# SerezD/vqvae-vqgan-pytorch-lightning

Measured on AMD Instinct MI355X. Metric: images/sec/node (256x256 bs=32/GPU) VQ-VAE train step, higher is better.
Workload: dtype bf16; 1 GPU; standard_vqvae cb=1024, 256x256 bs=32/GPU (encoder+VQ+decoder fwd/bwd + AdamW); yaml=example_confs/standard_vqvae.yaml, global_batch=32, parallelism=dp1, launch=hipGraph replay (fwd+bwd) + eager all-reduce + AdamW, deterministic=False

## Files before the change

### vqvae-vqgan-pytorch-lightning_amd/csrc/api.cpp

```cpp
#include <stdint.h>
#include <new>
#include "common.h"

extern "C" {

const char* vqk_status_str(int status) {
    switch (status) {
        case VQK_OK: return "ok";
        case VQK_ERR_SHAPE: return "unsupported or inconsistent shape";
        case VQK_ERR_DTYPE: return "unsupported dtype";
        case VQK_ERR_ALIGN: return "pointer is not 16-byte aligned";
        case VQK_ERR_LAUNCH: return "kernel launch failed";
        case VQK_ERR_ARG: return "bad argument";
        case VQK_ERR_WORKSPACE: return "workspace too small";
        default: return "unknown status";
    }
}

int vqk_version(void) { return 1; }
const char* vqk_arch(void) { return "gfx950"; }

}

struct vqk_ctx {
// ... 80 lines not shown
    {"FPROP_SPLITK", 0, 0},
    {"SK_BLOCKS", 0, 0},
    {"SK_MINSTEPS", 0, 0},
    {"SK_MAXMB", 0, 0},
    {"UPS_PHASE", 0, 0},
    {"WGRAD_BLOCKS", 0, 0},
    {"WGMX", 0, 0},
    {"WGRAD_GEN_BLOCKS", 0, 0},
    {"WGRAD_NO_PW16", 0, 0},
    {"WGRAD_NO_P16K", 0, 0},
    {"MX_HALF", 0, 0},
    {"MX_HALF_HW", 0, 0},
    {"UPFIRDN_TILE", 0, 0},
    {"GN_BLOCKS_REDUCE", 0, 0},
    {"GN_BLOCKS_APPLY", 0, 0},
    {"GN_NT_MB", 0, 0},
    {"GN_NO_SMALL", 0, 0},
    {"WGMX_COEF_E4", 0, 0},
    {"GN_CLUSTER_MAX_HW", 0, 0},
    {"COMM_CUS", 0, 0},
    {"MX_QUARTER", 0, 0},
    {"MX_S2", 0, 0},
    {"MX_S2_DGRAD_MIN", 0, 0},
    {"VQ_LDS", 0, 0},
    {"UPS_MERGE", 0, 0},
    {"TILE_QUEUE", 0, 0},
    {"X3_WL", 0, 0},
    {"X3_WGRAD_COEF_E4", 0, 0},
    {"X3_WGRAD_FOLD", 0, 0},
    {"X3_WGRAD_PHASE", 0, 0},
    {"X3_WGRAD_PHASE_CAP_PCT", 0, 0},
    {"X3_WGRAD_PHASE_COEF_E4", 0, 0},
    {"WGRAD_GROUP_LOAD_PCT", 0, 0},
    {"WGRAD_GROUP_MIN_PPS", 0, 0}
};
static constexpr int kTune = (int)(sizeof(g_tune) / sizeof(g_tune[0]));
TuneSlot* tune_slot(const char* name) {
    for (int i = 0; i < kTune; ++i)
        if (strcmp(g_tune[i].name, name) == 0) return &g_tune[i];
    abort();
}
}

extern "C" int vqk_set_tuning(const char* name, int value) {
    if (!name) return VQK_ERR_ARG;
    for (int i = 0; i < vqkd::kTune; ++i)
        if (strcmp(vqkd::g_tune[i].name, name) == 0) {
            __atomic_store_n(&vqkd::g_tune[i].value, value, __ATOMIC_RELAXED);
            __atomic_store_n(&vqkd::g_tune[i].is_set, 1, __ATOMIC_RELEASE);
            return VQK_OK;
        }
    return VQK_ERR_ARG;
}

extern "C" int vqk_reset_tuning(void) {
    for (int i = 0; i < vqkd::kTune; ++i) __atomic_store_n(&vqkd::g_tune[i].is_set, 0, __ATOMIC_RELAXED);
    return VQK_OK;
}

extern "C" int vqk_tuning_count(void) { return vqkd::kTune; }

extern "C" const char* vqk_tuning_name(int i) { return (i >= 0 && i < vqkd::kTune) ? vqkd::g_tune[i].name : nullptr; }
```

### vqvae-vqgan-pytorch-lightning_amd/csrc/conv.hip

```cpp
#include "conv_geom.h"
#include <type_traits>
#include <stdlib.h>
#include <math.h>

namespace {

using vqkd::ConvGeom;
using vqkd::xcd_remap;
using vqkd::pack_bf16x2;

__device__ __forceinline__ float epi_act(float v, int act) {
    if (act == 1) return tanhf(v);
    if (act == 2) return fmaxf(v, 0.0f);
    if (act == 3) return v > 0.0f ? v : 0.2f * v;
    return v;
}
__device__ __forceinline__ float epi_act_sel(float v, int act) {
    const float lo = act == 2 ? 0.0f : act == 3 ? 0.2f * v : v;
    return fmaxf(v, lo);
}


template <typename T> struct Mma;
template <> struct Mma<bf16_raw> {
// ... 975 lines not shown
                }
            }
        }
#pragma unroll
        for (int s5 = 0; s5 < 5; ++s5) a[s5] = an[s5];
    }
    if constexpr (STATS) {
        asm volatile("s_nop 3" : "+v"(sga), "+v"(sqa), "+v"(sgb), "+v"(sqb));
        sga += __shfl_xor(sga, 16, 64); sga += __shfl_xor(sga, 32, 64);
        sqa += __shfl_xor(sqa, 16, 64); sqa += __shfl_xor(sqa, 32, 64);
        sgb += __shfl_xor(sgb, 16, 64); sgb += __shfl_xor(sgb, 32, 64);
        sqb += __shfl_xor(sqb, 16, 64); sqb += __shfl_xor(sqb, 32, 64);
        if (lane < 16) {
            const int groups = g.cout >> 2;
            double* dst = g.gn_ws + ((int64_t)img_s * groups + ((cout_base >> 2) + 2 * lane)) * 2;
            atomicAdd(dst, (double)sga); atomicAdd(dst + 1, (double)sqa);
            atomicAdd(dst + 2, (double)sgb); atomicAdd(dst + 3, (double)sqb);
        }
    }
}

static thread_local int g_force_variant = CONV_VARIANT_AUTO;
#define g_det (vqkd::det_state().on)
#define g_det_ws (vqkd::det_state().ws)
#define g_det_ws_bytes (vqkd::det_state().bytes)
static thread_local int g_stream_blocks = 0;
static thread_local int g_wgrad_blocks = 0;

inline bool mx_shape_ok(const ConvGeom& g, int variant) {
    return VQK_TUNE("MX", 1) && variant != CONV_VARIANT_NO_MX && (g.cout & 127) == 0 && (g.cpt >> 2) >= 2 &&
           (int64_t)g.n * g.h_in * g.w_in * g.cin * 2 < 0x7fffffffLL && (int64_t)g.m * g.cout * 2 < 0x7fffffffLL;
}

inline bool mx_serves_1x1(const ConvGeom& g, int variant) {
    return mx_shape_ok(g, variant) && VQK_TUNE("MX_1X1", 1) && !g.ups;
}

inline int halo_twlog(const ConvGeom& g, int variant) {
    if ((g.ks != 3 && g.ks != 1) || (g.cpt % 8) != 0 || variant == CONV_VARIANT_IM2COL) return 0;
    if (g.ks == 1 && !mx_serves_1x1(g, variant)) return 0;
    const int prefer16 = VQK_TUNE("TW16", 0);
    if (prefer16 && (g.w % 16) == 0 && (g.h % 16) == 0) return 4;
    if ((g.w % 32) == 0 && (g.h % 8) == 0) return 5;
    if ((g.w % 16) == 0 && (g.h % 16) == 0) return 4;
    return 0;
}

inline bool fused_epilogue_serves(const ConvGeom& g, int variant) {
    return halo_twlog(g, variant) && (g.cout % 128) == 0 && variant != CONV_VARIANT_BREG && variant != CONV_VARIANT_PLAIN_WEIGHTS;
}

inline bool thin_f32_plain(const ConvGeom& g, int variant) {
    return g.ks == 3 && !g.ups && !g.zs && !g.sub && g.stride == 1 && g.pad == 1 && g.vh == g.h && g.vw == g.w &&
           variant != CONV_VARIANT_IM2COL;
}
inline bool thin_out_f32_serves(const ConvGeom& g, int variant) {
    return thin_f32_plain(g, variant) && g.cout == 4 && (g.cin % 16) == 0 && (g.h % 8) == 0 && (g.w % 32) == 0;
}
inline bool thin_in_f32_serves(const ConvGeom& g, int variant, bool has_res, int act) {
    return thin_f32_plain(g, variant) && g.cin == 4 && (g.cout == 64 || g.cout == 128 || g.cout == 256) && !has_res && act == 0 &&
           g.acc_scale == 1.0f && g.out_gain == 1.0f && g.w >= 4 && (g.w % 4) == 0 && (int64_t)(10) * (g.w + 2) * 16 <= 64 * 1024;
}

enum ConvForm : int {
    FORM_THIN_OUT_F32 = 0,
    FORM_THIN_IN_F32,
// ... 159 lines not shown
        launch_im2col<T, TO>(p, st, x, w, bias, res, y, zeros, g, act, skws);
        hipLaunchKernelGGL(conv_splitk_epilogue_kernel<TO>, dim3((unsigned)(((int64_t)g.m * g.cout / 4 + 255) / 256)), dim3(256), 0, st,
                           skws, bias, (const TO*)res, (TO*)y, g, act, p.splits);
        break;
    }
    default: return VQK_ERR_ARG;
    }
    if (hipGetLastError() != hipSuccess) return VQK_ERR_LAUNCH;
    return VQK_OK;
}

int launch_fprop_any(int dtype, int out_dtype, const void* x, const void* w, const float* bias, const void* res, void* y,
                     const void* zeros, const ConvGeom& g, int act, int wlayout, int variant, hipStream_t st) {
    if (dtype == VQK_F32 && out_dtype == VQK_F32) return launch_fprop<float, float>(x, w, bias, res, y, zeros, g, act, wlayout, variant, st);
    if (dtype == VQK_BF16 && out_dtype == VQK_BF16) return launch_fprop<bf16_raw, bf16_raw>(x, w, bias, res, y, zeros, g, act, wlayout, variant, st);
    if (dtype == VQK_BF16 && out_dtype == VQK_F32) return launch_fprop<bf16_raw, float>(x, w, bias, res, y, zeros, g, act, wlayout, variant, st);
    return VQK_ERR_DTYPE;
}

int make_geom(ConvGeom& g, int dtype, int n, int h_in, int w_in, int cin, int cout, int ksize, int ups) {
    if (dtype != VQK_F32 && dtype != VQK_BF16) return VQK_ERR_DTYPE;
    const int epc = dtype == VQK_F32 ? 4 : 8;
    if (n <= 0 || h_in <= 0 || w_in <= 0 || cin <= 0 || cout <= 0) return VQK_ERR_SHAPE;
    if (ksize != 1 && ksize != 3) return VQK_ERR_SHAPE;
    if (ups != 0 && ups != 1) return VQK_ERR_ARG;
    if (cin % epc) return VQK_ERR_SHAPE;
    g.n = n; g.h_in = h_in; g.w_in = w_in; g.h = h_in << ups; g.w = w_in << ups;
    g.cin = cin; g.cout = cout; g.ks = ksize; g.ups = ups;
    g.stride = 1; g.pad = ksize >> 1; g.zs = 0; g.vh = g.h; g.vw = g.w;
    g.acc_scale = 1.0f; g.out_gain = 1.0f; g.pool = 0; g.pool_scale = 1.0f;
    g.gn_ws = nullptr; g.gn_cpg = 0; g.gn_part_nblk = 0; g.gn_part_base = 0;
    g.act = 0; g.dy_pool = 0; g.tq = nullptr; g.tq_mode = 0; g.phase_rev = 0;
    g.ntap = ksize == 1 ? 1 : 9; g.tap_oy = g.tap_ox = 0; g.src_s = 1; g.src_a = g.src_b = 0; g.dst_s = 1; g.dst_a = g.dst_b = 0;
    g.tapw = 0; g.dst_h = g.dst_w = 0; g.s2 = 0; g.phase_mode = 0;
    g.fold = 0;
    const int64_t m = (int64_t)n * g.h * g.w;
    if (m > 0x7fffffff - 256) return VQK_ERR_SHAPE;
    g.m = (int)m;
    g.cpt = cin / epc;
    g.kchunks = ksize * ksize * g.cpt;
    g.wrow_chunks = g.kchunks; g.sub = 0;
    g.tiles_m = (g.m + 127) / 128;
    g.tiles_n = (cout + 127) / 128;
    return VQK_OK;
}

}

namespace vqkd {
int conv_make_geom(ConvGeom& g, int dtype, int n, int h_in, int w_in, int cin, int cout, int ksize, int ups) {
    return make_geom(g, dtype, n, h_in, w_in, cin, cout, ksize, ups);
}
int& conv_force_variant() { return g_force_variant; }
int& conv_wgrad_blocks() { return g_wgrad_blocks; }
}

extern "C" {

int vqk_conv_set_variant(int v) { g_force_variant = v; return VQK_OK; }
int vqk_conv_set_block_caps(int stream_blocks, int wgrad_blocks) {
    g_stream_blocks = stream_blocks; g_wgrad_blocks = wgrad_blocks;
    return VQK_OK;
}

static int conv_general(int dtype, const void* x, const void* w, const float* bias, const void* residual, void* y,
                        int out_dtype, int n, int h_in, int w_in, int cin, int cout, int ksize, int stride, int pad,
                        int mode, int h_out, int w_out, int act, float acc_scale, float out_gain, int wlayout,
// ... 178 lines not shown
        gx.gn_ws = gn_ws; gx.gn_cpg = cpg;
        return vqkd::launch_conv3x3_x3(x, w4, backward ? nullptr : bias, res, y, zeros, gx, 0, 0, vqk_stream(stream));
    }
    VQK_REQUIRE(!gn_ws || ((!backward || phase_rev) && groups > 0 && cout % groups == 0 && (cout / groups) % 4 == 0), VQK_ERR_SHAPE);
    VQK_REQUIRE(!res || (backward && phase_rev && vqk_aligned16(res)), VQK_ERR_ARG);
    ConvGeom g;
    const int rc = make_geom(g, dtype, n, h, w, cin, cout, 3, 0);
    if (rc) return rc;
    const int tw = halo_twlog(g, g_force_variant);
    const int mx_on = VQK_TUNE("MX", 1);
    const int ph_on = VQK_TUNE("UPS_PHASE", 1);
    VQK_REQUIRE(tw && mx_on && ph_on && (cout % 128) == 0 && (g.cpt >> 2) >= 2 && g_force_variant != CONV_VARIANT_NO_MX, VQK_ERR_SHAPE);
    VQK_REQUIRE((int64_t)4 * g.m * (backward ? cin : cout) * 2 < 0x7fffffffLL && (int64_t)g.m * (backward ? cout : cin) * 2 < 0x7fffffffLL,
                VQK_ERR_SHAPE);
    g.ntap = 4;
    const int64_t phase_elems = (int64_t)((cout + 127) / 128) * 128 * cin * 4;
    hipStream_t st = vqk_stream(stream);
    if (VQK_TUNE("UPS_MERGE", 1)) {
        ConvGeom gp = g;
        if (!backward) {
            gp.phase_mode = 1;
            gp.dst_s = 2;
            gp.phase_rev = phase_rev; gp.acc_scale = acc_scale;
            gp.gn_ws = gn_ws; gp.gn_cpg = gn_ws ? cout / groups : 0;
            if (gn_ws && g_det) { gp.gn_part_nblk = 4 * ((g.h * g.w) / 256); gp.gn_part_base = 0; }
        } else {
            gp.phase_mode = 2;
            gp.src_s = 2;
            gp.h_in = 2 * h; gp.w_in = 2 * w;
            gp.phase_rev = phase_rev; gp.acc_scale = acc_scale;
            gp.gn_ws = gn_ws; gp.gn_cpg = gn_ws ? cout / groups : 0;
            if (gn_ws && g_det) { gp.gn_part_nblk = (g.h * g.w) / 256; gp.gn_part_base = 0; }
        }
        return vqkd::launch_conv3x3_mx(x, w4, backward ? nullptr : bias, res, y, zeros, gp, tw, st);
    }
    for (int ph = 0; ph < 4; ++ph) {
        const int a = ph >> 1, b = ph & 1;
        ConvGeom gp = g;
        const void* res = nullptr;
        if (!backward) {
            gp.tap_oy = a; gp.tap_ox = b;
            gp.dst_s = 2; gp.dst_a = a; gp.dst_b = b;
            gp.gn_ws = gn_ws; gp.gn_cpg = gn_ws ? cout / groups : 0;
            if (gn_ws && g_det) { gp.gn_part_nblk = 4 * ((g.h * g.w) / 256); gp.gn_part_base = ph * ((g.h * g.w) / 256); }
        } else {
            gp.tap_oy = 1 - a; gp.tap_ox = 1 - b;
            gp.src_s = 2; gp.src_a = a; gp.src_b = b;
            gp.h_in = 2 * h; gp.w_in = 2 * w;
            res = ph ? y : nullptr;
        }
        const int r = vqkd::launch_conv3x3_mx(x, (const bf16_raw*)w4 + ph * phase_elems, backward ? nullptr : bias, res, y, zeros, gp, tw, st);
        if (r != VQK_OK) return r;
    }
    return VQK_OK;
}

static int s2_twlog(int h_out, int w_out, int pix) {
    if ((w_out % 32) == 0 && (h_out % (pix / 32)) == 0) return 5;
    if ((w_out % 16) == 0 && (h_out % (pix / 16)) == 0) return 4;
    return 0;
}

int vqk_conv2d_s2_supported(int dtype, int n, int h_out, int w_out, int cin, int cout, int backward) {
    if (dtype != VQK_BF16 || n <= 0 || h_out <= 0 || w_out <= 0 || cin <= 0 || cout <= 0) return 0;
    if (!VQK_TUNE("MX", 1) || !VQK_TUNE("MX_S2", 1) || g_force_variant == CONV_VARIANT_IM2COL || g_force_variant == CONV_VARIANT_NO_MX) return 0;
    const int64_t big = (int64_t)n * (2 * h_out + 1) * (2 * w_out + 1) * cin * 2, small = (int64_t)n * h_out * w_out * cout * 2;
    if (big >= 0x7fffffffLL || small >= 0x7fffffffLL) return 0;
    if (!backward) return (cin % 64) == 0 && (cout % 128) == 0 && s2_twlog(h_out, w_out, 128) != 0;
    return (cout % 64) == 0 && (cin % 128) == 0 && s2_twlog(h_out, w_out, 256) != 0 && w_out >= VQK_TUNE("MX_S2_DGRAD_MIN", 32);
}

int vqk_conv2d_s2_fprop(int dtype, const void* x, const void* wq, const float* bias, void* y, int n, int h_out, int w_out,
                        int cin, int cout, int act, float acc_scale, float out_gain, const void* zeros, void* stream) {
    VQK_REQUIRE(x && wq && y && zeros, VQK_ERR_ARG);
    VQK_REQUIRE(vqk_aligned16(x) && vqk_aligned16(wq) && vqk_aligned16(y), VQK_ERR_ALIGN);
    VQK_REQUIRE(act == 0 || act == 2 || act == 3, VQK_ERR_ARG);
    VQK_REQUIRE(vqk_conv2d_s2_supported(dtype, n, h_out, w_out, cin, cout, 0), VQK_ERR_SHAPE);
    ConvGeom g;
    const int rc = make_geom(g, dtype, n, h_out, w_out, cin, cout, 3, 0);
    if (rc) return rc;
    g.h_in = 2 * h_out + 1; g.w_in = 2 * w_out + 1;
    g.src_s = 2; g.s2 = 1;
    g.act = act; g.acc_scale = acc_scale; g.out_gain = out_gain;
// ... 132 lines not shown
```

### vqvae-vqgan-pytorch-lightning_amd/csrc/conv_geom.h

```cpp
#pragma once
#include "common.h"

namespace vqkd {

struct ConvGeom {
    int n, h_in, w_in, h, w, cin, cout, ks, ups;
    int stride, pad, zs, vh, vw;
    float acc_scale, out_gain;
    int pool;
    float pool_scale;
    int m;
    int sub, sub_py, sub_px, sub_h, sub_w, nkh, nkw, khl[2], kwl[2];
    int wrow_chunks;
    int cpt;
    int kchunks;
    int tiles_m, tiles_n;
    double* gn_ws;
    int gn_cpg;
    int gn_part_nblk, gn_part_base;
    int ntap, tap_oy, tap_ox, src_s, src_a, src_b, dst_s, dst_a, dst_b;
    int tapw, dst_h, dst_w, s2;
    int phase_mode;
    int phase_rev;
    int dy_pool;
    int act;
    int* tq;
    int tq_mode;
    int fold;
};

__device__ __forceinline__ int xcd_remap(int bid, int total) {
    const int q = total >> 3, r = total & 7, xcd = bid & 7, k = bid >> 3;
    return (xcd < r ? xcd * (q + 1) : r * (q + 1) + (xcd - r) * q) + k;
}

__device__ __forceinline__ unsigned pack_bf16x2(float a, float b) {
    typedef __attribute__((ext_vector_type(2))) float f32x2;
    typedef __attribute__((ext_vector_type(2))) __bf16 bf16x2_t;
    const f32x2 v = {a, b};
    return __builtin_bit_cast(unsigned, __builtin_convertvector(v, bf16x2_t));
}

int launch_conv3x3_mx(const void* x, const void* w, const float* bias, const void* res, void* y, const void* zeros,
                      const ConvGeom& g, int twlog, hipStream_t st);

int conv_make_geom(ConvGeom& g, int dtype, int n, int h_in, int w_in, int cin, int cout, int ksize, int ups);
}
enum ConvVariant : int {
    CONV_VARIANT_AUTO = -1,
    CONV_VARIANT_IM2COL = 0,
    CONV_VARIANT_HALO = 1,
    CONV_VARIANT_PLAIN_WEIGHTS = 2,
    CONV_VARIANT_BREG = 3,
    CONV_VARIANT_NO_HALF = 4,
    CONV_VARIANT_NO_MX = 5,
    CONV_VARIANT_MX = 6,
};
namespace vqkd {
int& conv_force_variant();
int& conv_wgrad_blocks();

bool conv3x3_x3_serves(const ConvGeom& g);
int launch_conv3x3_x3(const void* x, const void* w, const float* bias, const void* res, void* y, const void* zeros,
                      const ConvGeom& g, int act, int blocks_cap, hipStream_t st);
int launch_conv3x3_wgrad_x3(const void* x, const void* dy, float* dw, const ConvGeom& g, int blocks_cap, hipStream_t st);

int launch_conv3x3_thin_out_f32(const float* x, const float* w, const float* bias, const float* res, float* y, int n, int h, int wd,
                                int cin, int act, float acc_scale, float out_gain, hipStream_t st);
int launch_conv3x3_thin_in_f32(const float* x, const float* w, const float* bias, float* y, int n, int h, int wd, int cout, hipStream_t st);
int thin_wgrad_rows(int h, int w);
int launch_conv3x3_wgrad_thin_f32(int mode, const float* wide, const float* thin, float* dw, int n, int h, int w, int cw, float scale,
                                  hipStream_t st);

// ... 19 lines not shown
```

### vqvae-vqgan-pytorch-lightning_amd/csrc/conv_mx.hip

```cpp
#include "conv_geom.h"
#include <stdlib.h>

namespace {
using vqkd::ConvGeom;
using vqkd::pack_bf16x2;
using vqkd::xcd_remap;

#ifndef VQK_MX_RD
#define VQK_MX_RD 6
#endif
#ifndef VQK_MX_NT
#define VQK_MX_NT 2
#endif
#ifndef VQK_MX_HALO_AUX
#define VQK_MX_HALO_AUX 0
#endif
#ifndef VQK_MX_PRIO
#define VQK_MX_PRIO 0
#endif
#ifndef VQK_MX_PACE
#define VQK_MX_PACE 0
#endif
#ifndef VQK_MX_WL
#define VQK_MX_WL 0
#endif
#ifndef VQK_MX_JOUTER
#define VQK_MX_JOUTER 0
#endif
#ifndef VQK_MX_PIN
#define VQK_MX_PIN 1
#endif

#define SGB(mask, n) __builtin_amdgcn_sched_group_barrier(mask, n, 0)

__host__ __device__ constexpr int mx_tap_pix(bool s2, int tap, int twd, int hw2, int shp) {
    return s2 ? (((tap / 3) & 1) * 2 + ((tap % 3) & 1)) * shp + ((tap / 3) >> 1) * hw2 + ((tap % 3) >> 1)
              : (tap / twd) * hw2 + (tap % twd);
}

template <int TWLOG, bool POOL, int NTAP, int PIXELS = 256, int TAPW = 0, bool S2 = false>
__global__ __launch_bounds__(512, 2) void conv3x3_mx_kernel(const bf16_raw* __restrict__ x, const bf16_raw* __restrict__ wp,
                                                            const float* __restrict__ bias,
                                                            const bf16_raw* __restrict__ res, bf16_raw* __restrict__ y,
                                                            ConvGeom g) {
    constexpr int HM = NTAP == 1 ? 0 : 1;
    constexpr int PIX = PIXELS, TW = 1 << TWLOG, TH = PIX / TW;
    constexpr int HW2 = S2 ? TW + 1 : TW + 2 * HM;
    constexpr int SHP = (TH + 1) * (TW + 1);
    constexpr int HROWS = S2 ? 4 * SHP : (TH + 2 * HM) * HW2;
    constexpr int RS = 80;
    constexpr int PIECES = (HROWS * 5 + 63) / 64;
    constexpr int NBUF = S2 ? 2 : 3;
    constexpr int BUF = PIECES * 1024, STG = NBUF * BUF, SPITCH = 272, SCR = STG + PIX * SPITCH;
    constexpr int TQR = SCR + 1024;
    constexpr int TWD = TAPW ? TAPW : NTAP == 9 ? 3 : NTAP == 4 ? 2 : 1;
    constexpr int NI = VQK_MX_WL ? PIX / 32 : PIX / 64, NJ = VQK_MX_WL ? 1 : 2;
    constexpr int NQ = PIX / 16;
    static_assert(PIX == 256 || ((PIX == 128 || PIX == 64) && !POOL && NTAP == 9), "256-pixel tiles, or plain 128- / 64-pixel part tiles");
    constexpr int NPH = NTAP * 2;
    static_assert(NTAP == 9 || ((NTAP == 4 || NTAP == 2 || NTAP == 1) && !POOL), "3x3 taps, the 2x2 / 1x2 / 2x1 taps of a phase, or a 1x1 conv");
    static_assert(!S2 || (NTAP == 9 && !POOL && PIX == 128), "stride 2: 3x3 taps, 128-pixel tiles");
    static_assert(TAPW == 0 || (NTAP == 2 && (TAPW == 1 || TAPW == 2)), "TAPW names the orientation of a 2-tap window");
    constexpr int XS = (PIECES + 3) / 4;
    constexpr int OOB = (int)0x80000000;
    typedef bf16x8_t frag_t;
    typedef __attribute__((ext_vector_type(4))) unsigned int u32x4;
    typedef __attribute__((ext_vector_type(2))) unsigned int u32x2;
    extern __shared__ __attribute__((aligned(16))) char smem[];

    const int tid = threadIdx.x, lane = tid & 63;
    const int wave = __builtin_amdgcn_readfirstlane(tid >> 6);
    const int tiles_x = g.w >> TWLOG, tiles_y = g.h / TH;
    const int pmode = NTAP == 4 ? g.phase_mode : 0;
    const int total_tiles = g.n * tiles_y * tiles_x * g.tiles_n * (pmode == 1 ? 4 : 1);
    const int nch = g.cpt >> 2;
    const int nun = pmode == 2 ? 4 * nch : nch;
    const int grid = (int)gridDim.x, q8 = grid >> 3, r8 = grid & 7, xcd = (int)blockIdx.x & 7;
    const int cnt = q8 + (xcd < r8 ? 1 : 0);
    const int c0 = xcd < r8 ? xcd * (q8 + 1) : r8 * (q8 + 1) + (xcd - r8) * q8;
    const int vbid = c0 + ((int)blockIdx.x >> 3);
    if (vbid >= total_tiles) return;
    auto tile_of = [&](int k) -> int { const int j = k / cnt; return c0 + (k - j * cnt) + j * grid; };
    const int tqm = g.tq ? g.tq_mode : 0;
    volatile VQK_LDS int* const ring = (volatile VQK_LDS int*)(smem + TQR);
    auto next_id = [&](int j) -> int { return tqm ? __builtin_amdgcn_readfirstlane(ring[j & 7]) : vbid + j * grid; };
    const bool pro_sync = tqm == 2 || (tqm && nun < 4);

    struct TilePos { int img, py0, px0, nt, ph; };
    auto tile_pos = [&](int t) -> TilePos {
        TilePos tp;
        tp.nt = t % g.tiles_n; t /= g.tiles_n;
        tp.ph = 0;
        if (pmode == 1) { tp.ph = t & 3; t >>= 2; }
        const int txi = t % tiles_x; t /= tiles_x;
        const int tyi = t % tiles_y;
        tp.img = t / tiles_y; tp.py0 = tyi * TH; tp.px0 = txi * TW;
        return tp;
    };
    auto unit_barrier = [&]() { asm volatile("s_waitcnt lgkmcnt(0)\n\ts_barrier" ::: "memory"); };
    double* const gnws = g.gn_ws;

    if (wave < 4) {
        if (VQK_MX_PRIO) __builtin_amdgcn_s_setprio(VQK_MX_PRIO);
        const int wm = VQK_MX_WL ? 0 : wave >> 1, wn = VQK_MX_WL ? wave : wave & 1;
        const int p = lane & 31, kg = lane >> 5;
        unsigned abase[NI], sbase[NI];
#pragma unroll
        for (int i = 0; i < NI; ++i) {
            int ty, tx;
            if (TWLOG == 5) { ty = wm * NI + i; tx = p; }
            else { ty = wm * 2 * NI + 2 * i + (p >> 4); tx = p & 15; }
            abase[i] = (unsigned)(((ty + (pmode ? 0 : g.tap_oy)) * HW2 + tx + (pmode ? 0 : g.tap_ox)) * RS + kg * 16);
            sbase[i] = (unsigned)(STG + (ty * TW + tx) * SPITCH + (wn * (32 * NJ) + 4 * kg) * 2);
        }
        const int lane16 = lane * 16;
        const int phase_bytes = (g.cout >> 5) * nch * (NPH * 1024);
        const __amdgpu_buffer_rsrc_t wsrd = __builtin_amdgcn_make_buffer_rsrc(
            const_cast<bf16_raw*>(wp), 0, phase_bytes * (pmode ? 4 : 1), 0x00020000);
        auto unit_ph = [&](int key, int c) -> int { return pmode == 2 ? c / nch : (key >> 16); };
        auto unit_w = [&](int key, int c, int j) -> int {
            const int ph = unit_ph(key, c), cc = pmode == 2 ? c - ph * nch : c;
            const int wph = (NTAP == 4 && g.phase_rev) ? 3 - ph : ph;
            return wph * phase_bytes + (((key & 0xffff) * 4 + wn * NJ + j) * nch + cc) * (NPH * 1024);
        };
        auto phase_off = [&](int ph) -> int {
            const int a = ph >> 1, b = ph & 1;
            return pmode == 1 ? (a * HW2 + b) * RS : pmode == 2 ? ((1 - a) * HW2 + (1 - b)) * RS : 0;
        };
        auto tile_nt = [&](int t) -> int {
            return (t % g.tiles_n) | (pmode == 1 ? ((t / g.tiles_n) & 3) << 16 : 0);
        };
        auto wload = [&](int soff) -> frag_t {
            return __builtin_bit_cast(frag_t, __builtin_amdgcn_raw_buffer_load_b128(wsrd, lane16, soff, 0));
        };

        constexpr int RD = NTAP == 9 ? VQK_MX_RD : NTAP == 4 ? 4 : 2;
        static_assert(NPH % RD == 0, "weight ring depth must divide the phases of a unit");
        f32x16 acc[NI][NJ];
        frag_t bw[RD][NJ];
        int wcur[NJ];
        if (pro_sync) unit_barrier();
        const int t_first = tqm == 2 ? __builtin_amdgcn_readfirstlane(ring[0]) : vbid;
        if (t_first >= total_tiles) return;
        int cur_nt = tile_nt(t_first);
#pragma unroll
        for (int j = 0; j < NJ; ++j) wcur[j] = unit_w(cur_nt, 0, j);
#pragma unroll
        for (int d = 0; d < RD; ++d)
#pragma unroll
            for (int j = 0; j < NJ; ++j) bw[d][j] = wload(wcur[j] + d * 1024);
        unit_barrier();

        int tj = 0, c = 0, bi = 0, t_next = 0;
        for (;;) {
            if (c == nun - 2) t_next = next_id(tj + 1);
            const bool last_c = c == nun - 1, more = last_c && t_next < total_tiles;
            int nc = c + 1, nxt_nt = cur_nt;
            if (last_c) {
                if (more) { nc = 0; nxt_nt = tile_nt(t_next); }
                else nc = c;
            }
            int wnxt[NJ];
#pragma unroll
            for (int j = 0; j < NJ; ++j) wnxt[j] = unit_w(nxt_nt, nc, j);
            const char* lbase[NI];
#pragma unroll
            for (int i = 0; i < NI; ++i) lbase[i] = smem + bi * BUF + abase[i] + (NTAP == 4 ? phase_off(unit_ph(cur_nt, c)) : 0);

            frag_t a[2][NI];
#pragma unroll
            for (int i = 0; i < NI; ++i) a[0][i] = *reinterpret_cast<const frag_t*>(lbase[i]);
            __builtin_amdgcn_sched_barrier(0);
#pragma unroll
            for (int tap = 0; tap < NTAP; ++tap) {
                const int toff = mx_tap_pix(S2, tap, TWD, HW2, SHP) * RS;
#pragma unroll
                for (int ks = 0; ks < 2; ++ks) {
                    const bool reads = ks == 0 || tap < NTAP - 1;
                    const int ph = tap * 2 + ks;
                    if (ks == 0) {
#pragma unroll
                        for (int i = 0; i < NI; ++i) a[1][i] = *reinterpret_cast<const frag_t*>(lbase[i] + toff + 32);
                    } else if (tap < NTAP - 1) {
                        const int toff1 = mx_tap_pix(S2, tap + 1, TWD, HW2, SHP) * RS;
#pragma unroll
                        for (int i = 0; i < NI; ++i) a[0][i] = *reinterpret_cast<const frag_t*>(lbase[i] + toff1);
                    }
                    if (tap == 0 && ks == 0 && c == 0) {
                        const f32x16 zero = {0.f, 0.f, 0.f, 0.f, 0.f, 0.f, 0.f, 0.f, 0.f, 0.f, 0.f, 0.f, 0.f, 0.f, 0.f, 0.f};
#pragma unroll
                        for (int i = 0; i < NI; ++i)
#pragma unroll
                            for (int j = 0; j < NJ; ++j)
                                acc[i][j] = __builtin_amdgcn_mfma_f32_32x32x16_bf16(bw[ph % RD][j], a[ks][i], zero, 0, 0, 0);
                    } else if (VQK_MX_JOUTER) {
#pragma unroll
                        for (int j = 0; j < NJ; ++j)
#pragma unroll
                            for (int i = 0; i < NI; ++i)
                                acc[i][j] = __builtin_amdgcn_mfma_f32_32x32x16_bf16(bw[ph % RD][j], a[ks][i], acc[i][j], 0, 0, 0);
                    } else {
#pragma unroll
                        for (int i = 0; i < NI; ++i)
#pragma unroll
                            for (int j = 0; j < NJ; ++j)
                                acc[i][j] = __builtin_amdgcn_mfma_f32_32x32x16_bf16(bw[ph % RD][j], a[ks][i], acc[i][j], 0, 0, 0);
                    }
#pragma unroll
                    for (int j = 0; j < NJ; ++j) {
                        const int soff = (ph + RD >= NPH) ? wnxt[j] + (ph + RD - NPH) * 1024 : wcur[j] + (ph + RD) * 1024;
                        bw[ph % RD][j] = wload(soff);
                    }
                    if (VQK_MX_PIN) {
                        if (reads) {
#pragma unroll
                            for (int i = 0; i < NI; ++i) { SGB(0x008, 1); SGB(0x100, 1); }
                            if constexpr (NI * NJ - NI > 0) SGB(0x008, NI * NJ - NI);
                        } else {
                            SGB(0x008, NI * NJ);
                        }
                        SGB(0x020, NJ);
// ... 4 lines not shown
            if (c == nun - 1) {
#pragma unroll
                for (int i = 0; i < NI; ++i)
#pragma unroll
                    for (int j = 0; j < NJ; ++j)
#pragma unroll
                        for (int rq = 0; rq < 4; ++rq) {
                            const u32x2 o = {pack_bf16x2(acc[i][j][4 * rq], acc[i][j][4 * rq + 1]),
                                             pack_bf16x2(acc[i][j][4 * rq + 2], acc[i][j][4 * rq + 3])};
                            *reinterpret_cast<u32x2*>(smem + sbase[i] + (j * 32 + 8 * rq) * 2) = o;
                        }
            }
            unit_barrier();
            if (last_c) { if (!more) break; ++tj; }
            cur_nt = nxt_nt; c = nc;
            bi = bi == NBUF - 1 ? 0 : bi + 1;
#pragma unroll
            for (int j = 0; j < NJ; ++j) wcur[j] = wnxt[j];
        }
        return;
    }

    const int xt = tid - 256, xw = wave - 4;
    const __amdgpu_buffer_rsrc_t xsrd = __builtin_amdgcn_make_buffer_rsrc(
        const_cast<bf16_raw*>(x), 0, (int)((int64_t)g.n * g.h_in * g.w_in * g.cin * 2), 0x00020000);
    const int out_bytes = (int)((int64_t)g.n * g.dst_h * g.dst_w * g.cout * 2);
    const __amdgpu_buffer_rsrc_t rsrd = __builtin_amdgcn_make_buffer_rsrc(const_cast<bf16_raw*>(res), 0, res ? out_bytes : 0, 0x00020000);
    const __amdgpu_buffer_rsrc_t ysrd = __builtin_amdgcn_make_buffer_rsrc(y, 0, out_bytes >> (POOL ? 2 : 0), 0x00020000);

    int rel[XS], flg[XS];
#pragma unroll
    for (int sl = 0; sl < XS; ++sl) {
        const int s = (xw + 4 * sl) * 64 + lane;
        const int hp = s / 5, cp = s - hp * 5;
        if constexpr (S2) {
            const int sh = hp / SHP, q = hp - sh * SHP;
            const int hy = q / HW2, hx = q - hy * HW2, pa = sh >> 1, pb = sh & 1;
            rel[sl] = (((2 * hy + pa) * g.w_in + 2 * hx + pb) * g.cin + cp * 8) * 2;
            flg[sl] = (cp == 4 || hp >= HROWS || (pa && hy == TH) || (pb && hx == TW)) ? 16 : 0;
        } else {
            const int hy = hp / HW2, hx = hp - hy * HW2;
            rel[sl] = (((((hy - HM) * g.src_s) >> g.ups) * g.w_in + (((hx - HM) * g.src_s) >> g.ups)) * g.cin + cp * 8) * 2;
            flg[sl] = (HM && hy == 0 ? 1 : 0) | (HM && hy == TH + 1 ? 2 : 0) | (HM && hx == 0 ? 4 : 0) | (HM && hx == TW + 1 ? 8 : 0) |
                      ((cp == 4 || hp >= HROWS) ? 16 : 0);
        }
    }
    auto issue_halo = [&](const TilePos& tp, int cu, int bufi) {
        const int uph = pmode == 2 ? cu / nch : 0, c = pmode == 2 ? cu - uph * nch : cu;
        const int sa = pmode == 2 ? (uph >> 1) : g.src_a, sb = pmode == 2 ? (uph & 1) : g.src_b;
        const int base = (((tp.img * g.h_in + ((tp.py0 * g.src_s + sa) >> g.ups)) * g.w_in + ((tp.px0 * g.src_s + sb) >> g.ups)) * g.cin + c * 32) * 2;
        const int tb = S2 ? 16 : ((tp.py0 == 0 ? 1 : 0) | (tp.py0 + TH == g.h ? 2 : 0) | (tp.px0 == 0 ? 4 : 0) | (tp.px0 + TW == g.w ? 8 : 0) | 16);
#pragma unroll
        for (int sl = 0; sl < XS; ++sl) {
            if (xw + 4 * sl < PIECES) {
                const int off = (flg[sl] & tb) ? OOB : base + rel[sl];
                __builtin_amdgcn_raw_ptr_buffer_load_lds(
                    xsrd, (VQK_LDS void*)(smem + bufi * BUF + (xw + 4 * sl) * 1024), 16,
                    off, 0, 0, VQK_MX_HALO_AUX);
            }
        }
    };
    auto unpack8 = [&](const u32x4& r, float (&v)[8]) {
#pragma unroll
        for (int e = 0; e < 4; ++e) { v[2 * e] = __uint_as_float(r[e] << 16); v[2 * e + 1] = __uint_as_float(r[e] & 0xffff0000u); }
    };
    auto pack8 = [&](const float (&v)[8]) -> u32x4 {
        const u32x4 o = {pack_bf16x2(v[0], v[1]), pack_bf16x2(v[2], v[3]), pack_bf16x2(v[4], v[5]), pack_bf16x2(v[6], v[7])};
        return o;
    };
    const int slot = xt & 15;
    constexpr int NP = POOL ? 4 : NQ;
    constexpr int NR = NQ;
    struct OutPos { int pix0, ppix0, co, img, tile; };
    auto out_pos = [&](const TilePos& tp) -> OutPos {
        OutPos o;
        o.tile = (tp.py0 / TH) * tiles_x + (tp.px0 >> TWLOG) + (pmode == 1 ? tp.ph * tiles_y * tiles_x : 0);
        const int da = pmode == 1 ? (tp.ph >> 1) : g.dst_a, db = pmode == 1 ? (tp.ph & 1) : g.dst_b;
        o.pix0 = (tp.img * g.dst_h + tp.py0 * g.dst_s + da) * g.dst_w + tp.px0 * g.dst_s + db;
        o.ppix0 = (tp.img * (g.h >> 1) + (tp.py0 >> 1)) * (g.w >> 1) + (tp.px0 >> 1);
        o.co = tp.nt * 128 + slot * 8;
        o.img = tp.img;
        return o;
    };
    auto res_off = [&](const OutPos& o, int k) -> int {
// ... 260 lines not shown
                       (bf16_raw*)y, g);
    return hipGetLastError() == hipSuccess ? VQK_OK : VQK_ERR_LAUNCH;
}

int device_cus() {
    static const int cus = [] {
        int dev = 0, n = 0;
        if (hipGetDevice(&dev) != hipSuccess ||
            hipDeviceGetAttribute(&n, hipDeviceAttributeMultiprocessorCount, dev) != hipSuccess || n <= 0) n = 256;
        return n;
    }();
    return cus;
}
}

int launch_conv3x3_mx(const void* x, const void* w, const float* bias, const void* res, void* y, const void* zeros,
                      const ConvGeom& g_in, int twlog, hipStream_t st) {
    (void)zeros;
    ConvGeom g = g_in;
    if (!g.dst_h) { g.dst_h = g.h * g.dst_s; g.dst_w = g.w * g.dst_s; }
    const int half_on = VQK_TUNE("MX_HALF", 1);
    const int half_hw = VQK_TUNE("MX_HALF_HW", 256);
    const bool half = half_on && g.h * g.w <= half_hw && !g.pool && g.ntap == 9 && (twlog == 4 ? (g.h % 8) == 0 : (g.h % 4) == 0);
    const int qmode = VQK_TUNE("MX_QUARTER", 1);
    const bool quarter = half && qmode && (g.tiles_n <= 2 || qmode >= 2) && (twlog == 4 ? (g.h % 4) == 0 : (g.h % 2) == 0);
    const int th = (quarter ? 64 : half ? 128 : 256) >> twlog;
    const int total = g.n * (g.h / th) * (g.w >> twlog) * g.tiles_n * ((g.ntap == 4 && g.phase_mode == 1) ? 4 : 1);
    int cus = device_cus() - VQK_TUNE("COMM_CUS", 0);
    if (cus < 1) cus = 1;
    const dim3 grid((unsigned)(total < cus ? total : cus));
    const int tqm = VQK_TUNE("TILE_QUEUE", 0);
    const DetState& tqs = tile_queue_state();
    auto set_queue = [&](int tiles, int blocks) {
        const bool on = tqm > 0 && tqs.ws != nullptr && tqs.bytes >= 64 && tiles > blocks && (g.cpt >> 2) >= 2;
        g.tq = on ? reinterpret_cast<int*>(tqs.ws) : nullptr;
        g.tq_mode = on ? (tqm >= 2 ? 2 : 1) : 0;
    };
    set_queue(total, (int)grid.x);
    constexpr int TQB = 64;
    constexpr int lds5 = 3 * (((256 / 32 + 2) * 34 * 5 + 63) / 64) * 1024 + 256 * 272 + 1024 + TQB;
    constexpr int lds4 = 3 * (((256 / 16 + 2) * 18 * 5 + 63) / 64) * 1024 + 256 * 272 + 1024 + TQB;
    constexpr int lds4h = 3 * (((128 / 16 + 2) * 18 * 5 + 63) / 64) * 1024 + 128 * 272 + 1024 + TQB;
    constexpr int lds5h = 3 * (((128 / 32 + 2) * 34 * 5 + 63) / 64) * 1024 + 128 * 272 + 1024 + TQB;
#define MXL(K, L) return mx_launch<K>(grid, L, st, x, w, bias, res, y, g)
    constexpr int lds4q = 3 * (((64 / 16 + 2) * 18 * 5 + 63) / 64) * 1024 + 64 * 272 + 1024 + TQB;
    constexpr int lds5q = 3 * (((64 / 32 + 2) * 34 * 5 + 63) / 64) * 1024 + 64 * 272 + 1024 + TQB;
    if (g.s2) {
        constexpr int lds5s = 2 * ((4 * (128 / 32 + 1) * 33 * 5 + 63) / 64) * 1024 + 128 * 272 + 1024 + TQB;
        constexpr int lds4s = 2 * ((4 * (128 / 16 + 1) * 17 * 5 + 63) / 64) * 1024 + 128 * 272 + 1024 + TQB;
        if (g.pool || g.ntap != 9 || (twlog == 4 ? (g.h % 8) : (g.h % 4)) != 0) return VQK_ERR_ARG;
        const int tot2 = g.n * (g.h / (128 >> twlog)) * (g.w >> twlog) * g.tiles_n;
        const dim3 grid2((unsigned)(tot2 < cus ? tot2 : cus));
        set_queue(tot2, (int)grid2.x);
        if (twlog == 5) return mx_launch<conv3x3_mx_kernel<5, false, 9, 128, 0, true>>(grid2, lds5s, st, x, w, bias, res, y, g);
        return mx_launch<conv3x3_mx_kernel<4, false, 9, 128, 0, true>>(grid2, lds4s, st, x, w, bias, res, y, g);
    }
    if (g.ntap == 2) {
        if (g.pool) return VQK_ERR_ARG;
        if (g.tapw == 2) { if (twlog == 5) MXL((conv3x3_mx_kernel<5, false, 2, 256, 2>), lds5); else MXL((conv3x3_mx_kernel<4, false, 2, 256, 2>), lds4); }
        if (g.tapw == 1) { if (twlog == 5) MXL((conv3x3_mx_kernel<5, false, 2, 256, 1>), lds5); else MXL((conv3x3_mx_kernel<4, false, 2, 256, 1>), lds4); }
        return VQK_ERR_ARG;
    }
    if (quarter) {
        if (twlog == 5) MXL((conv3x3_mx_kernel<5, false, 9, 64>), lds5q); else MXL((conv3x3_mx_kernel<4, false, 9, 64>), lds4q);
    } else if (half) {
        if (twlog == 5) MXL((conv3x3_mx_kernel<5, false, 9, 128>), lds5h); else MXL((conv3x3_mx_kernel<4, false, 9, 128>), lds4h);
    } else if (g.ntap == 4) {
        if (g.pool) return VQK_ERR_ARG;
        if (twlog == 5) MXL((conv3x3_mx_kernel<5, false, 4>), lds5); else MXL((conv3x3_mx_kernel<4, false, 4>), lds4);
    } else if (g.ntap == 1) {
        if (g.pool) return VQK_ERR_ARG;
        constexpr int lds1 = 3 * ((256 * 5 + 63) / 64) * 1024 + 256 * 272 + 1024 + TQB;
        if (twlog == 5) MXL((conv3x3_mx_kernel<5, false, 1>), lds1); else MXL((conv3x3_mx_kernel<4, false, 1>), lds1);
    } else if (twlog == 5) {
        if (g.pool) MXL((conv3x3_mx_kernel<5, true, 9>), lds5); else MXL((conv3x3_mx_kernel<5, false, 9>), lds5);
    } else {
        if (g.pool) MXL((conv3x3_mx_kernel<4, true, 9>), lds4); else MXL((conv3x3_mx_kernel<4, false, 9>), lds4);
    }
#undef MXL
}

}
```

Before: 1178 images/sec.

## Stage 64-channel units with trimmed halos in 2x2-tap phase upsample convs

Adds a U64 variant of the MX conv kernel for the 2x2-tap phase-decomposed (upsample) convolutions. Each staged unit now holds 64 input channels instead of 32, and the halo is trimmed to (TH+1)x(TW+1) by folding the phase offset into the global address. Two buffers replace three. This halves the number of pipeline stages and barriers per tile and cuts redundant halo loads, at the cost of deeper buffering per stage and fewer buffers for overlapping loads with compute. The variant is on by default through a new tuning knob.

```diff
diff --git a/vqvae-vqgan-pytorch-lightning_amd/csrc/api.cpp b/vqvae-vqgan-pytorch-lightning_amd/csrc/api.cpp
--- a/vqvae-vqgan-pytorch-lightning_amd/csrc/api.cpp
+++ b/vqvae-vqgan-pytorch-lightning_amd/csrc/api.cpp
@@ -136,7 +136,8 @@
     {"X3_WGRAD_PHASE_CAP_PCT", 0, 0},
     {"X3_WGRAD_PHASE_COEF_E4", 0, 0},
     {"WGRAD_GROUP_LOAD_PCT", 0, 0},
-    {"WGRAD_GROUP_MIN_PPS", 0, 0}
+    {"WGRAD_GROUP_MIN_PPS", 0, 0},
+    {"MX_PHASE_U64", 0, 0}
 };
 static constexpr int kTune = (int)(sizeof(g_tune) / sizeof(g_tune[0]));
 TuneSlot* tune_slot(const char* name) {
diff --git a/vqvae-vqgan-pytorch-lightning_amd/csrc/conv.hip b/vqvae-vqgan-pytorch-lightning_amd/csrc/conv.hip
--- a/vqvae-vqgan-pytorch-lightning_amd/csrc/conv.hip
+++ b/vqvae-vqgan-pytorch-lightning_amd/csrc/conv.hip
@@ -1031,6 +1031,12 @@
            (int64_t)g.n * g.h_in * g.w_in * g.cin * 2 < 0x7fffffffLL && (int64_t)g.m * g.cout * 2 < 0x7fffffffLL;
 }
 
+inline bool mx_phase_u64_serves(const ConvGeom& g, int tw) {
+    const int units = (g.cin / 64) * (g.phase_mode == 2 ? 4 : 1);
+    return VQK_TUNE("MX_PHASE_U64", 1) && g.ntap == 4 && (g.cin % 64) == 0 && units >= 2 && (tw == 4 || tw == 5) &&
+           vqkd::mx_phase_u64_lds(tw) <= vqkd::MX_LDS_MAX;
+}
+
 inline bool mx_serves_1x1(const ConvGeom& g, int variant) {
     return mx_shape_ok(g, variant) && VQK_TUNE("MX_1X1", 1) && !g.ups;
 }
@@ -1256,7 +1262,7 @@
     g.gn_ws = nullptr; g.gn_cpg = 0; g.gn_part_nblk = 0; g.gn_part_base = 0;
     g.act = 0; g.dy_pool = 0; g.tq = nullptr; g.tq_mode = 0; g.phase_rev = 0;
     g.ntap = ksize == 1 ? 1 : 9; g.tap_oy = g.tap_ox = 0; g.src_s = 1; g.src_a = g.src_b = 0; g.dst_s = 1; g.dst_a = g.dst_b = 0;
-    g.tapw = 0; g.dst_h = g.dst_w = 0; g.s2 = 0; g.phase_mode = 0;
+    g.tapw = 0; g.dst_h = g.dst_w = 0; g.s2 = 0; g.phase_mode = 0; g.unit64 = 0;
     g.fold = 0;
     const int64_t m = (int64_t)n * g.h * g.w;
     if (m > 0x7fffffff - 256) return VQK_ERR_SHAPE;
@@ -1501,6 +1507,7 @@
             gp.gn_ws = gn_ws; gp.gn_cpg = gn_ws ? cout / groups : 0;
             if (gn_ws && g_det) { gp.gn_part_nblk = (g.h * g.w) / 256; gp.gn_part_base = 0; }
         }
+        gp.unit64 = mx_phase_u64_serves(gp, tw);
         return vqkd::launch_conv3x3_mx(x, w4, backward ? nullptr : bias, res, y, zeros, gp, tw, st);
     }
     for (int ph = 0; ph < 4; ++ph) {
@@ -1518,6 +1525,7 @@
             gp.h_in = 2 * h; gp.w_in = 2 * w;
             res = ph ? y : nullptr;
         }
+        gp.unit64 = mx_phase_u64_serves(gp, tw);
         const int r = vqkd::launch_conv3x3_mx(x, (const bf16_raw*)w4 + ph * phase_elems, backward ? nullptr : bias, res, y, zeros, gp, tw, st);
         if (r != VQK_OK) return r;
     }
diff --git a/vqvae-vqgan-pytorch-lightning_amd/csrc/conv_geom.h b/vqvae-vqgan-pytorch-lightning_amd/csrc/conv_geom.h
--- a/vqvae-vqgan-pytorch-lightning_amd/csrc/conv_geom.h
+++ b/vqvae-vqgan-pytorch-lightning_amd/csrc/conv_geom.h
@@ -15,6 +15,7 @@
     int cpt;
     int kchunks;
     int tiles_m, tiles_n;
+    int unit64;
     double* gn_ws;
     int gn_cpg;
     int gn_part_nblk, gn_part_base;
@@ -39,6 +40,11 @@
     typedef __attribute__((ext_vector_type(2))) __bf16 bf16x2_t;
     const f32x2 v = {a, b};
     return __builtin_bit_cast(unsigned, __builtin_convertvector(v, bf16x2_t));
+}
+
+constexpr int MX_LDS_MAX = 160 * 1024;
+constexpr int mx_phase_u64_lds(int twlog) {
+    return 2 * ((((256 >> twlog) + 1) * ((1 << twlog) + 1) * 9 + 63) / 64) * 1024 + 256 * 272 + 1024 + 64;
 }
 
 int launch_conv3x3_mx(const void* x, const void* w, const float* bias, const void* res, void* y, const void* zeros,
diff --git a/vqvae-vqgan-pytorch-lightning_amd/csrc/conv_mx.hip b/vqvae-vqgan-pytorch-lightning_amd/csrc/conv_mx.hip
--- a/vqvae-vqgan-pytorch-lightning_amd/csrc/conv_mx.hip
+++ b/vqvae-vqgan-pytorch-lightning_amd/csrc/conv_mx.hip
@@ -38,26 +38,29 @@
               : (tap / twd) * hw2 + (tap % twd);
 }
 
-template <int TWLOG, bool POOL, int NTAP, int PIXELS = 256, int TAPW = 0, bool S2 = false>
+template <int TWLOG, bool POOL, int NTAP, int PIXELS = 256, int TAPW = 0, bool S2 = false, bool U64 = false>
 __global__ __launch_bounds__(512, 2) void conv3x3_mx_kernel(const bf16_raw* __restrict__ x, const bf16_raw* __restrict__ wp,
                                                             const float* __restrict__ bias,
                                                             const bf16_raw* __restrict__ res, bf16_raw* __restrict__ y,
                                                             ConvGeom g) {
     constexpr int HM = NTAP == 1 ? 0 : 1;
     constexpr int PIX = PIXELS, TW = 1 << TWLOG, TH = PIX / TW;
-    constexpr int HW2 = S2 ? TW + 1 : TW + 2 * HM;
+    constexpr int CPU = U64 ? 2 : 1;
+    constexpr int HW2 = (S2 || U64) ? TW + 1 : TW + 2 * HM;
     constexpr int SHP = (TH + 1) * (TW + 1);
-    constexpr int HROWS = S2 ? 4 * SHP : (TH + 2 * HM) * HW2;
-    constexpr int RS = 80;
-    constexpr int PIECES = (HROWS * 5 + 63) / 64;
-    constexpr int NBUF = S2 ? 2 : 3;
+    constexpr int HROWS = S2 ? 4 * SHP : U64 ? SHP : (TH + 2 * HM) * HW2;
+    constexpr int SPP = 4 * CPU + 1;
+    constexpr int RS = SPP * 16;
+    constexpr int PIECES = (HROWS * SPP + 63) / 64;
+    constexpr int NBUF = (S2 || U64) ? 2 : 3;
+    static_assert(!U64 || (NTAP == 4 && PIXELS == 256 && !S2), "64-channel units: the 2x2-tap phase forms");
     constexpr int BUF = PIECES * 1024, STG = NBUF * BUF, SPITCH = 272, SCR = STG + PIX * SPITCH;
     constexpr int TQR = SCR + 1024;
     constexpr int TWD = TAPW ? TAPW : NTAP == 9 ? 3 : NTAP == 4 ? 2 : 1;
     constexpr int NI = VQK_MX_WL ? PIX / 32 : PIX / 64, NJ = VQK_MX_WL ? 1 : 2;
     constexpr int NQ = PIX / 16;
     static_assert(PIX == 256 || ((PIX == 128 || PIX == 64) && !POOL && NTAP == 9), "256-pixel tiles, or plain 128- / 64-pixel part tiles");
-    constexpr int NPH = NTAP * 2;
+    constexpr int NPH = NTAP * 2 * CPU;
     static_assert(NTAP == 9 || ((NTAP == 4 || NTAP == 2 || NTAP == 1) && !POOL), "3x3 taps, the 2x2 / 1x2 / 2x1 taps of a phase, or a 1x1 conv");
     static_assert(!S2 || (NTAP == 9 && !POOL && PIX == 128), "stride 2: 3x3 taps, 128-pixel tiles");
     static_assert(TAPW == 0 || (NTAP == 2 && (TAPW == 1 || TAPW == 2)), "TAPW names the orientation of a 2-tap window");
@@ -73,7 +76,7 @@
     const int tiles_x = g.w >> TWLOG, tiles_y = g.h / TH;
     const int pmode = NTAP == 4 ? g.phase_mode : 0;
     const int total_tiles = g.n * tiles_y * tiles_x * g.tiles_n * (pmode == 1 ? 4 : 1);
-    const int nch = g.cpt >> 2;
+    const int nch = (g.cpt >> 2) / CPU;
     const int nun = pmode == 2 ? 4 * nch : nch;
     const int grid = (int)gridDim.x, q8 = grid >> 3, r8 = grid & 7, xcd = (int)blockIdx.x & 7;
     const int cnt = q8 + (xcd < r8 ? 1 : 0);
@@ -110,7 +113,7 @@
             int ty, tx;
             if (TWLOG == 5) { ty = wm * NI + i; tx = p; }
             else { ty = wm * 2 * NI + 2 * i + (p >> 4); tx = p & 15; }
-            abase[i] = (unsigned)(((ty + (pmode ? 0 : g.tap_oy)) * HW2 + tx + (pmode ? 0 : g.tap_ox)) * RS + kg * 16);
+            abase[i] = (unsigned)(((ty + ((pmode || U64) ? 0 : g.tap_oy)) * HW2 + tx + ((pmode || U64) ? 0 : g.tap_ox)) * RS + kg * 16);
             sbase[i] = (unsigned)(STG + (ty * TW + tx) * SPITCH + (wn * (32 * NJ) + 4 * kg) * 2);
         }
         const int lane16 = lane * 16;
@@ -125,7 +128,7 @@
         };
         auto phase_off = [&](int ph) -> int {
             const int a = ph >> 1, b = ph & 1;
-            return pmode == 1 ? (a * HW2 + b) * RS : pmode == 2 ? ((1 - a) * HW2 + (1 - b)) * RS : 0;
+            return U64 ? 0 : pmode == 1 ? (a * HW2 + b) * RS : pmode == 2 ? ((1 - a) * HW2 + (1 - b)) * RS : 0;
         };
         auto tile_nt = [&](int t) -> int {
             return (t % g.tiles_n) | (pmode == 1 ? ((t / g.tiles_n) & 3) << 16 : 0);
@@ -172,21 +175,27 @@
             for (int i = 0; i < NI; ++i) a[0][i] = *reinterpret_cast<const frag_t*>(lbase[i]);
             __builtin_amdgcn_sched_barrier(0);
 #pragma unroll
+            for (int cu = 0; cu < CPU; ++cu)
+#pragma unroll
             for (int tap = 0; tap < NTAP; ++tap) {
-                const int toff = mx_tap_pix(S2, tap, TWD, HW2, SHP) * RS;
+                const int toff = mx_tap_pix(S2, tap, TWD, HW2, SHP) * RS + cu * 64;
 #pragma unroll
                 for (int ks = 0; ks < 2; ++ks) {
-                    const bool reads = ks == 0 || tap < NTAP - 1;
-                    const int ph = tap * 2 + ks;
+                    const bool reads = ks == 0 || tap < NTAP - 1 || cu < CPU - 1;
+                    const int ph = (cu * NTAP + tap) * 2 + ks;
                     if (ks == 0) {
 #pragma unroll
                         for (int i = 0; i < NI; ++i) a[1][i] = *reinterpret_cast<const frag_t*>(lbase[i] + toff + 32);
                     } else if (tap < NTAP - 1) {
-                        const int toff1 = mx_tap_pix(S2, tap + 1, TWD, HW2, SHP) * RS;
+                        const int toff1 = mx_tap_pix(S2, tap + 1, TWD, HW2, SHP) * RS + cu * 64;
+#pragma unroll
+                        for (int i = 0; i < NI; ++i) a[0][i] = *reinterpret_cast<const frag_t*>(lbase[i] + toff1);
+                    } else if (cu < CPU - 1) {
+                        const int toff1 = mx_tap_pix(S2, 0, TWD, HW2, SHP) * RS + (cu + 1) * 64;
 #pragma unroll
                         for (int i = 0; i < NI; ++i) a[0][i] = *reinterpret_cast<const frag_t*>(lbase[i] + toff1);
                     }
-                    if (tap == 0 && ks == 0 && c == 0) {
+                    if (cu == 0 && tap == 0 && ks == 0 && c == 0) {
                         const f32x16 zero = {0.f, 0.f, 0.f, 0.f, 0.f, 0.f, 0.f, 0.f, 0.f, 0.f, 0.f, 0.f, 0.f, 0.f, 0.f, 0.f};
 #pragma unroll
                         for (int i = 0; i < NI; ++i)
@@ -257,24 +266,28 @@
 #pragma unroll
     for (int sl = 0; sl < XS; ++sl) {
         const int s = (xw + 4 * sl) * 64 + lane;
-        const int hp = s / 5, cp = s - hp * 5;
+        const int hp = s / SPP, cp = s - hp * SPP;
         if constexpr (S2) {
             const int sh = hp / SHP, q = hp - sh * SHP;
             const int hy = q / HW2, hx = q - hy * HW2, pa = sh >> 1, pb = sh & 1;
             rel[sl] = (((2 * hy + pa) * g.w_in + 2 * hx + pb) * g.cin + cp * 8) * 2;
-            flg[sl] = (cp == 4 || hp >= HROWS || (pa && hy == TH) || (pb && hx == TW)) ? 16 : 0;
+            flg[sl] = (cp == SPP - 1 || hp >= HROWS || (pa && hy == TH) || (pb && hx == TW)) ? 16 : 0;
         } else {
             const int hy = hp / HW2, hx = hp - hy * HW2;
             rel[sl] = (((((hy - HM) * g.src_s) >> g.ups) * g.w_in + (((hx - HM) * g.src_s) >> g.ups)) * g.cin + cp * 8) * 2;
-            flg[sl] = (HM && hy == 0 ? 1 : 0) | (HM && hy == TH + 1 ? 2 : 0) | (HM && hx == 0 ? 4 : 0) | (HM && hx == TW + 1 ? 8 : 0) |
-                      ((cp == 4 || hp >= HROWS) ? 16 : 0);
+            constexpr int HB = U64 ? TH : TH + 1, HR = U64 ? TW : TW + 1;
+            flg[sl] = (HM && hy == 0 ? 1 : 0) | (HM && hy == HB ? 2 : 0) | (HM && hx == 0 ? 4 : 0) | (HM && hx == HR ? 8 : 0) |
+                      ((cp == SPP - 1 || hp >= HROWS) ? 16 : 0);
         }
     }
     auto issue_halo = [&](const TilePos& tp, int cu, int bufi) {
         const int uph = pmode == 2 ? cu / nch : 0, c = pmode == 2 ? cu - uph * nch : cu;
         const int sa = pmode == 2 ? (uph >> 1) : g.src_a, sb = pmode == 2 ? (uph & 1) : g.src_b;
-        const int base = (((tp.img * g.h_in + ((tp.py0 * g.src_s + sa) >> g.ups)) * g.w_in + ((tp.px0 * g.src_s + sb) >> g.ups)) * g.cin + c * 32) * 2;
-        const int tb = S2 ? 16 : ((tp.py0 == 0 ? 1 : 0) | (tp.py0 + TH == g.h ? 2 : 0) | (tp.px0 == 0 ? 4 : 0) | (tp.px0 + TW == g.w ? 8 : 0) | 16);
+        const int oy = !U64 ? 0 : pmode == 1 ? (tp.ph >> 1) : pmode == 2 ? 1 - (uph >> 1) : g.tap_oy;
+        const int ox = !U64 ? 0 : pmode == 1 ? (tp.ph & 1) : pmode == 2 ? 1 - (uph & 1) : g.tap_ox;
+        const int base = (((tp.img * g.h_in + (((tp.py0 + oy) * g.src_s + sa) >> g.ups)) * g.w_in + (((tp.px0 + ox) * g.src_s + sb) >> g.ups)) * g.cin + c * (32 * CPU)) * 2;
+        const int tb = S2 ? 16 : ((tp.py0 == 0 && (!U64 || oy == 0) ? 1 : 0) | (tp.py0 + TH == g.h && (!U64 || oy == 1) ? 2 : 0) |
+                                  (tp.px0 == 0 && (!U64 || ox == 0) ? 4 : 0) | (tp.px0 + TW == g.w && (!U64 || ox == 1) ? 8 : 0) | 16);
 #pragma unroll
         for (int sl = 0; sl < XS; ++sl) {
             if (xw + 4 * sl < PIECES) {
@@ -601,7 +614,8 @@
     const int tqm = VQK_TUNE("TILE_QUEUE", 0);
     const DetState& tqs = tile_queue_state();
     auto set_queue = [&](int tiles, int blocks) {
-        const bool on = tqm > 0 && tqs.ws != nullptr && tqs.bytes >= 64 && tiles > blocks && (g.cpt >> 2) >= 2;
+        const int units = (g.cpt >> 2) / ((g.ntap == 4 && g.unit64) ? 2 : 1) * ((g.ntap == 4 && g.phase_mode == 2) ? 4 : 1);
+        const bool on = tqm > 0 && tqs.ws != nullptr && tqs.bytes >= 64 && tiles > blocks && units >= 2;
         g.tq = on ? reinterpret_cast<int*>(tqs.ws) : nullptr;
         g.tq_mode = on ? (tqm >= 2 ? 2 : 1) : 0;
     };
@@ -636,6 +650,13 @@
         if (twlog == 5) MXL((conv3x3_mx_kernel<5, false, 9, 128>), lds5h); else MXL((conv3x3_mx_kernel<4, false, 9, 128>), lds4h);
     } else if (g.ntap == 4) {
         if (g.pool) return VQK_ERR_ARG;
+        if (g.unit64) {
+            constexpr int lds5u = mx_phase_u64_lds(5), lds4u = mx_phase_u64_lds(4);
+            static_assert(lds5u <= MX_LDS_MAX && lds4u <= MX_LDS_MAX, "two trimmed 144-byte halo buffers fit beside the staging tile");
+            if ((g.cin & 63) != 0 || (g.cpt >> 3) * (g.phase_mode == 2 ? 4 : 1) < 2) return VQK_ERR_ARG;
+            if (twlog == 5) MXL((conv3x3_mx_kernel<5, false, 4, 256, 0, false, true>), lds5u);
+            else MXL((conv3x3_mx_kernel<4, false, 4, 256, 0, false, true>), lds4u);
+        }
         if (twlog == 5) MXL((conv3x3_mx_kernel<5, false, 4>), lds5); else MXL((conv3x3_mx_kernel<4, false, 4>), lds4);
     } else if (g.ntap == 1) {
         if (g.pool) return VQK_ERR_ARG;
```

After: 1196 images/sec, median of 6. +1.6%, better.
